# hyye/lio-mapping

Hardware: AMD Instinct MI355X
Metric: sliding-window solves/sec, 64-line 130k-pt scans, window=15 (opt_window=5) (higher is better)
Workload: dtype f64 (solve) / f32 (features); 1 GPU; HDL-64E outdoor_test_config_64, S_outdoor ray-cast scans, window_size=15 opt_window_size=5, one SolveOptimization per step, clouds resident in HBM; n_lidar_residuals=78236, local_map_points=76752, surf_stack_points=19386, parallelism=1 window

## Files before the change

### lio-mapping_amd/csrc/cloud_kernels.h

```cpp
#pragma once
#include <cstdint>

#include "dev.h"

namespace lio {

struct VoxParams {
  float mn[3], mx[3];
  int minb[3], divb[3];
  int overflow;
  int n_valid;
};

struct Affine3f { float m[12]; };

#define LIO_MAX_FRAMES 32

struct ConcatSeg { const float4 *src; int n; int dst_off; int set_intensity; float intensity; Affine3f tf; int identity; };
struct ConcatArgs { ConcatSeg seg[LIO_MAX_FRAMES]; int nseg; int total; };
void launch_transform_concat(const ConcatArgs &a, float4 *dst, hipStream_t s);

void launch_deskew_to_end(float4 *pts, int n, const float q[4], const float p[3], float time_factor, hipStream_t s);

void launch_cloud_bounds(const float4 *pts, int n, DBuf<float> &partial, VoxParams *d_out, hipStream_t s);

class VoxelGridDev {
 public:
  size_t run(const float4 *in, size_t n, float leaf, DBuf<float4> &out, hipStream_t s, VoxParams *host_params = nullptr);
  void launch(const float4 *in, size_t n, float leaf, DBuf<float4> &out, hipStream_t s);
  size_t finish(VoxParams *host_params = nullptr);
  void set_host_signal(bool on) { use_signal_ = on; }
  VoxelGridDev() = default;
  VoxelGridDev(const VoxelGridDev &) = delete;
  VoxelGridDev &operator=(const VoxelGridDev &) = delete;
  ~VoxelGridDev();

 private:
  const float4 *p_in_ = nullptr; size_t p_n_ = 0; DBuf<float4> *p_out_ = nullptr; hipStream_t p_stream_ = nullptr;
  float p_leaf_ = 0.f;
  void enqueue(bool exact);
  int *h_count_ = nullptr;
  VoxParams *h_params_ = nullptr;
  DBuf<float> partial_;
  DBuf<VoxParams> params_;
  DBuf<uint32_t> keys_, keys2_, vals_, vals2_;
  DBuf<int> count_, tile_heads_;
  DBuf<char> tmp_;
  unsigned *h_flag_ = nullptr;
  unsigned seq_ = 0;
  HostSignal sig_{};
  bool use_signal_ = true;
};
bool host_signal_enabled();

struct GridDesc {
  int origin[3];
  int dims[3];
  float inv_cell;
  int n_points;
};

class KnnGrid {
 public:
  void build(const float4 *pts, size_t n, const float mn[3], const float mx[3], float cell, hipStream_t s);
  const float4 *sorted() const { return sorted_.p; }
  const int *cells() const { return cells_.p; }
  const GridDesc &desc() const { return desc_; }

 private:
  GridDesc desc_{};
  DBuf<uint32_t> keys_, keys2_, vals_, vals2_;
  DBuf<float4> sorted_;
  DBuf<int> cells_, cnt_;
  bool cnt_dirty_ = false;
  DBuf<char> tmp_;
};

struct FeatFrame { const float4 *stack; int M; int slot_off; int tf_index; const uint32_t *order = nullptr; };
struct FeatArgs {
  FeatFrame fr[LIO_MAX_FRAMES];
  int nframes;
  int max_M;
  float min_match_sq_dis, min_plane_dis;
  int mapping_mode;
  float fixed_pz[3];
};
void launch_features(const FeatArgs &a, const float *transforms, const float4 *map_sorted, const int *cells, const GridDesc &g,
                     uint8_t *valid, float4 *coef, float *score, const int *skip_flag, hipStream_t s, float4 *abs_coef = nullptr);

void launch_line_features(const float4 *stack, int M, int slot_off, const float *transform, const float fixed_pz[3], float min_match_sq_dis,
                          const float4 *map_sorted, const int *cells, const GridDesc &g, uint8_t *valid, float4 *coef,
                          const int *skip_flag, hipStream_t s);

void launch_knn(const float4 *query, int m, int k, float radius_sq, const float4 *map_sorted, const int *cells, const GridDesc &g,
                int32_t *idx, float *sqd, hipStream_t s);

void launch_map_round(const FeatArgs &surf, const float4 *corner_stack, int Mc, const float *transform, const float4 *corner_map,
                      const int *corner_cells, const GridDesc &corner_grid, const float4 *surf_map, const int *surf_cells,
                      const GridDesc &surf_grid, uint8_t *valid, float4 *coef, float4 *abs_coef, const int *skip_flag, hipStream_t s);

struct SolveSetup {
  float tf[LIO_MAX_FRAMES][8];
  int ntf;
  float odom_T[8];
  int set_odom;
};
struct OdomState;
void launch_solve_setup(const SolveSetup &a, float *d_transforms, OdomState *d_odom, uint8_t *valid, size_t n_valid, hipStream_t s);
// ... 61 lines not shown
```

### lio-mapping_amd/csrc/cloud_kernels.hip

```cpp
#include <cstring>
#include <hip/hip_runtime.h>
#include <rocprim/rocprim.hpp>

#include <cfloat>
#include <climits>

#include "cloud_kernels.h"
#include "cloud_device.h"

namespace lio {

__global__ void k_transform_concat(ConcatArgs a, float4 *__restrict__ dst) {
  int gid = blockIdx.x * blockDim.x + threadIdx.x;
  if (gid >= a.total) return;
  int sidx = 0;
  for (int k = 1; k < a.nseg; ++k)
    if (gid >= a.seg[k].dst_off) sidx = k;
  const ConcatSeg &sg = a.seg[sidx];
  int local = gid - sg.dst_off;
  float4 p = sg.src[local];
  float4 o;
  if (sg.identity) {
    o = p;
  } else {
    const float *m = sg.tf.m;
    o.x = m[0] * p.x + m[1] * p.y + m[2] * p.z + m[3];
    o.y = m[4] * p.x + m[5] * p.y + m[6] * p.z + m[7];
    o.z = m[8] * p.x + m[9] * p.y + m[10] * p.z + m[11];
    o.w = p.w;
  }
  if (sg.set_intensity) o.w = sg.intensity;
  dst[gid] = o;
}

void launch_transform_concat(const ConcatArgs &a, float4 *dst, hipStream_t s) {
  if (a.total <= 0) return;
  hipLaunchKernelGGL(k_transform_concat, dim3(cdiv(a.total, 256)), dim3(256), 0, s, a, dst);
  LIO_HIP(hipGetLastError());
}

__global__ void k_deskew_to_end(float4 *pts, int n, Quat<float> qe, Vec3<float> te, float time_factor) {
// ... 48 lines not shown
  float mn[3] = {FLT_MAX, FLT_MAX, FLT_MAX}, mx[3] = {-FLT_MAX, -FLT_MAX, -FLT_MAX};
  float cnt = 0;
  for (int b = t; b < nb; b += 256) {
    for (int d = 0; d < 3; ++d) { mn[d] = fminf(mn[d], partial[b * 8 + d]); mx[d] = fmaxf(mx[d], partial[b * 8 + 3 + d]); }
    cnt += partial[b * 8 + 6];
  }
  for (int d = 0; d < 3; ++d) { sm[d][t] = mn[d]; sm[3 + d][t] = mx[d]; }
  sm[6][t] = cnt;
  __syncthreads();
  for (int st = 128; st > 0; st >>= 1) {
    if (t < st) {
      for (int d = 0; d < 3; ++d) { sm[d][t] = fminf(sm[d][t], sm[d][t + st]); sm[3 + d][t] = fmaxf(sm[3 + d][t], sm[3 + d][t + st]); }
      sm[6][t] += sm[6][t + st];
    }
    __syncthreads();
  }
  if (t != 0) return;
  for (int d = 0; d < 3; ++d) { mn[d] = sm[d][0]; mx[d] = sm[3 + d][0]; }
  cnt = sm[6][0];
  VoxParams v;
  long long dd[3];
  for (int d = 0; d < 3; ++d) {
    v.mn[d] = mn[d]; v.mx[d] = mx[d];
    dd[d] = (long long)((mx[d] - mn[d]) * inv_leaf) + 1;
    v.minb[d] = int(floorf(mn[d] * inv_leaf));
    int maxb = int(floorf(mx[d] * inv_leaf));
    v.divb[d] = maxb - v.minb[d] + 1;
  }
  v.overflow = (cnt > 0 && dd[0] * dd[1] * dd[2] > (long long)INT_MAX) ? 1 : 0;
  v.n_valid = int(cnt);
  *out = v;
}

__global__ void k_vox_keys(const float4 *__restrict__ pts, int n, float inv_leaf, const VoxParams *__restrict__ vp,
                           uint32_t *__restrict__ keys, uint32_t *__restrict__ vals) {
  int i = blockIdx.x * blockDim.x + threadIdx.x;
  if (i >= n) return;
  float4 p = pts[i];
  uint32_t key = 0xFFFFFFFFu;
  if (finite3(p)) {
    int i0 = int(floorf(p.x * inv_leaf) - float(vp->minb[0]));
    int i1 = int(floorf(p.y * inv_leaf) - float(vp->minb[1]));
    int i2 = int(floorf(p.z * inv_leaf) - float(vp->minb[2]));
    key = uint32_t(i0 + i1 * vp->divb[0] + i2 * vp->divb[0] * vp->divb[1]);
  }
  keys[i] = key;
  vals[i] = uint32_t(i);
}

#define VOX_KEY_THREADS 256
__global__ void __launch_bounds__(VOX_KEY_THREADS) k_vox_keys_abs(const float4 *__restrict__ pts, int n, float inv_leaf, uint32_t *__restrict__ keys,
                                                                 uint32_t *__restrict__ vals, float *__restrict__ partial, int *__restrict__ range_overflow) {
  const int i = blockIdx.x * VOX_KEY_THREADS + threadIdx.x;
  float mn[3] = {FLT_MAX, FLT_MAX, FLT_MAX}, mx[3] = {-FLT_MAX, -FLT_MAX, -FLT_MAX};
  float cnt = 0;
  if (i < n) {
    const float4 p = pts[i];
    uint32_t key = 0xFFFFFFFFu;
    if (finite3(p)) {
      cnt = 1.f;
      mn[0] = mx[0] = p.x; mn[1] = mx[1] = p.y; mn[2] = mx[2] = p.z;
      const float cx = floorf(p.x * inv_leaf), cy = floorf(p.y * inv_leaf), cz = floorf(p.z * inv_leaf);
      if (fabsf(cx) < 1024.f && fabsf(cy) < 1024.f && fabsf(cz) < 511.f) key = (uint32_t(int(cz) + 512) << 22) | (uint32_t(int(cy) + 1024) << 11) | uint32_t(int(cx) + 1024);
      else *range_overflow = 1;
    }
    keys[i] = key;
    vals[i] = uint32_t(i);
  }
  __shared__ float sm[7][VOX_KEY_THREADS / 64];
  const int lane = threadIdx.x & 63, wv = threadIdx.x >> 6;
#pragma unroll
  for (int o = 32; o > 0; o >>= 1) {
    for (int d = 0; d < 3; ++d) { mn[d] = fminf(mn[d], __shfl_xor(mn[d], o, 64)); mx[d] = fmaxf(mx[d], __shfl_xor(mx[d], o, 64)); }
    cnt += __shfl_xor(cnt, o, 64);
  }
  if (lane == 0) { for (int d = 0; d < 3; ++d) { sm[d][wv] = mn[d]; sm[3 + d][wv] = mx[d]; } sm[6][wv] = cnt; }
  __syncthreads();
  if (threadIdx.x < 7) {
    const int t = threadIdx.x;
    float v = sm[t][0];
    for (int w = 1; w < VOX_KEY_THREADS / 64; ++w) v = t < 3 ? fminf(v, sm[t][w]) : (t < 6 ? fmaxf(v, sm[t][w]) : v + sm[t][w]);
    partial[size_t(blockIdx.x) * 8 + t] = v;
  }
}

#define VOX_TILE 256
__device__ __forceinline__ bool vox_is_head(const uint32_t *__restrict__ keys, int i, int n, uint32_t k) {
  return i < n && k != 0xFFFFFFFFu && (i == 0 || keys[i - 1] != k);
}
__global__ void __launch_bounds__(VOX_TILE) k_vox_tile_heads(const uint32_t *__restrict__ keys, int n, int *__restrict__ tile_heads,
                                                             const float *__restrict__ partial, int npartial, float inv_leaf, VoxParams *__restrict__ params) {
  if (blockIdx.x == gridDim.x - 1) {
    if (npartial <= 0) return;
    __shared__ float sm[7][VOX_TILE];
    const int t = threadIdx.x;
    float mn[3] = {FLT_MAX, FLT_MAX, FLT_MAX}, mx[3] = {-FLT_MAX, -FLT_MAX, -FLT_MAX};
    float cnt = 0;
    for (int b = t; b < npartial; b += VOX_TILE) {
      for (int d = 0; d < 3; ++d) { mn[d] = fminf(mn[d], partial[size_t(b) * 8 + d]); mx[d] = fmaxf(mx[d], partial[size_t(b) * 8 + 3 + d]); }
      cnt += partial[size_t(b) * 8 + 6];
    }
    for (int d = 0; d < 3; ++d) { sm[d][t] = mn[d]; sm[3 + d][t] = mx[d]; }
    sm[6][t] = cnt;
    __syncthreads();
    for (int st = VOX_TILE / 2; st > 0; st >>= 1) {
      if (t < st) {
        for (int d = 0; d < 3; ++d) { sm[d][t] = fminf(sm[d][t], sm[d][t + st]); sm[3 + d][t] = fmaxf(sm[3 + d][t], sm[3 + d][t + st]); }
        sm[6][t] += sm[6][t + st];
      }
      __syncthreads();
    }
    if (t != 0) return;
    VoxParams v;
    long long dd[3];
    for (int d = 0; d < 3; ++d) {
      v.mn[d] = sm[d][0]; v.mx[d] = sm[3 + d][0];
// ... 62 lines not shown
    int g = base_i + VOX_TILE;
    while (g < n && keys[g] == k) { const float4 p = pts[vals[g]]; ax += p.x; ay += p.y; az += p.z; ai += p.w; ++g; ++cnt; }
  }
  const float c = float(cnt);
  out[pos] = make_float4(ax / c, ay / c, az / c, ai / c);
}

void launch_cloud_bounds(const float4 *pts, int n, DBuf<float> &partial, VoxParams *d_out, hipStream_t s) {
  const int nb = std::max(1, std::min(cdiv(n, 256), 512));
  partial.reserve(size_t(nb) * 8);
  hipLaunchKernelGGL(k_bounds_partial, dim3(nb), dim3(256), 0, s, pts, n, partial.p);
  hipLaunchKernelGGL(k_bounds_final, dim3(1), dim3(256), 0, s, partial.p, nb, 1.0f, d_out);
  LIO_HIP(hipGetLastError());
}

bool host_signal_enabled() {
  static const bool on = [] { const char *e = std::getenv("LIO_HOST_SIGNAL"); return e ? std::atoi(e) != 0 : true; }();
  return on;
}

void VoxelGridDev::launch(const float4 *in, size_t n, float leaf, DBuf<float4> &out, hipStream_t s) {
  p_in_ = in; p_n_ = n; p_out_ = &out; p_stream_ = s; p_leaf_ = leaf;
  if (n == 0) return;
  enqueue(false);
}

void VoxelGridDev::enqueue(bool exact) {
  const float4 *in = p_in_;
  const size_t n = p_n_;
  DBuf<float4> &out = *p_out_;
  hipStream_t s = p_stream_;
  const int ni = int(n);
  const float inv_leaf = 1.0f / p_leaf_;
  const int nkb = cdiv(ni, VOX_KEY_THREADS);
  partial_.reserve(size_t(std::max(nkb, 512)) * 8);
  params_.reserve(1);
  keys_.reserve(n); keys2_.reserve(n); vals_.reserve(n); vals2_.reserve(n);
  if (count_.cap < 2) { count_.reserve(2); LIO_HIP(hipMemsetAsync(count_.p, 0, count_.cap * sizeof(int), s)); }
  out.reserve(n);
  if (!h_count_) {
    LIO_HIP(hipHostMalloc(reinterpret_cast<void **>(&h_count_), 256, hipHostMallocCoherent));
    static_assert(sizeof(VoxMail) <= 128, "mailbox layout");
    std::memset(h_count_, 0, 256);
    h_params_ = reinterpret_cast<VoxParams *>(h_count_ + 1);
    h_flag_ = reinterpret_cast<unsigned *>(reinterpret_cast<char *>(h_count_) + 128);
  }
  int *d_range = count_.p + 1;
  const bool use_sig = use_signal_ && host_signal_enabled();
  if (!use_sig) LIO_HIP(hipMemsetAsync(d_range, 0, sizeof(int), s));
  int npartial = 0;
  if (exact) {
    const int nb = std::min(cdiv(ni, 256), 512);
    hipLaunchKernelGGL(k_bounds_partial, dim3(nb), dim3(256), 0, s, in, ni, partial_.p);
    hipLaunchKernelGGL(k_bounds_final, dim3(1), dim3(256), 0, s, partial_.p, nb, inv_leaf, params_.p);
    hipLaunchKernelGGL(k_vox_keys, dim3(cdiv(ni, 256)), dim3(256), 0, s, in, ni, inv_leaf, params_.p, keys_.p, vals_.p);
  } else {
    hipLaunchKernelGGL(k_vox_keys_abs, dim3(nkb), dim3(VOX_KEY_THREADS), 0, s, in, ni, inv_leaf, keys_.p, vals_.p, partial_.p, d_range);
    npartial = nkb;
  }
  size_t tmp_bytes = 0;
  LIO_HIP(rocprim::radix_sort_pairs(nullptr, tmp_bytes, keys_.p, keys2_.p, vals_.p, vals2_.p, n, 0, 32, s));
  tmp_.reserve(tmp_bytes + 256);
  LIO_HIP(rocprim::radix_sort_pairs(tmp_.p, tmp_bytes, keys_.p, keys2_.p, vals_.p, vals2_.p, n, 0, 32, s));
  const int ntiles = cdiv(ni, VOX_TILE);
  tile_heads_.reserve(ntiles);
  hipLaunchKernelGGL(k_vox_tile_heads, dim3(ntiles + 1), dim3(VOX_TILE), 0, s, keys2_.p, ni, tile_heads_.p, partial_.p, npartial, inv_leaf, params_.p);
  sig_ = HostSignal();
  if (use_sig) { sig_.flag = h_flag_; sig_.seq = ++seq_; }

  hipLaunchKernelGGL(k_vox_centroids, dim3(ntiles), dim3(VOX_TILE), 0, s, in, keys2_.p, vals2_.p, tile_heads_.p, ni, out.p, count_.p, params_.p, d_range,
                     reinterpret_cast<VoxMail *>(h_count_), sig_);
  LIO_HIP(hipGetLastError());
  if (!sig_.flag) {
    VoxMail *m = reinterpret_cast<VoxMail *>(h_count_);
    LIO_HIP(hipMemcpyAsync(&m->count, count_.p, sizeof(int), hipMemcpyDeviceToHost, s));
    LIO_HIP(hipMemcpyAsync(&m->params, params_.p, sizeof(VoxParams), hipMemcpyDeviceToHost, s));
    LIO_HIP(hipMemcpyAsync(&m->range_overflow, d_range, sizeof(int), hipMemcpyDeviceToHost, s));
  }
}

size_t VoxelGridDev::finish(VoxParams *host_params) {
  if (p_n_ == 0) {
    if (host_params) std::memset(host_params, 0, sizeof(*host_params));
    return 0;
  }
  const VoxMail *m = reinterpret_cast<const VoxMail *>(h_count_);
  bool redone = false;
  for (;;) {
    if (sig_.flag) wait_host_signal(sig_, p_stream_);
    else LIO_HIP(hipStreamSynchronize(p_stream_));
    if (m->range_overflow == 1 && !redone) {
      enqueue(true);
      redone = true;
      continue;
    }
    if (redone) LIO_HIP(hipStreamSynchronize(p_stream_));
    break;
  }
  int count = m->count;
  const VoxParams hp = m->params;
  if (hp.overflow) {
    p_out_->reserve(p_n_);
    LIO_HIP(hipMemcpyAsync(p_out_->p, p_in_, p_n_ * sizeof(float4), hipMemcpyDeviceToDevice, p_stream_));
// ... 29 lines not shown

__global__ void k_cell_place(const float4 *__restrict__ pts, const uint32_t *__restrict__ keys, const uint32_t *__restrict__ slot, int n,
                             const int *__restrict__ starts, float4 *__restrict__ sorted, int *__restrict__ cnt) {
  int i = blockIdx.x * blockDim.x + threadIdx.x;
  if (i >= n) return;
  float4 p = pts[i];
  p.w = __int_as_float(i);
  const uint32_t c = keys[i];
  sorted[starts[c] + int(slot[i])] = p;
  cnt[c] = 0;
}

void KnnGrid::build(const float4 *pts, size_t n, const float mn[3], const float mx[3], float cell, hipStream_t s) {
  desc_.inv_cell = 1.0f / cell;
  desc_.n_points = int(n);
  size_t ncells = 1;
  for (int d = 0; d < 3; ++d) {
    int lo = int(std::floor(mn[d] * desc_.inv_cell)) - 1;
    int hi = int(std::floor(mx[d] * desc_.inv_cell)) + 1;
    desc_.origin[d] = lo;
    desc_.dims[d] = hi - lo + 1;
    ncells *= size_t(desc_.dims[d]);
  }
  if (ncells > (size_t(1) << 30)) throw DeviceError("KnnGrid: cell table too large");
  cells_.reserve(ncells + 1);
  if (cnt_.cap < ncells + 1 || cnt_dirty_) {
    cnt_.reserve(ncells + 1);
    LIO_HIP(hipMemsetAsync(cnt_.p, 0, cnt_.cap * sizeof(int), s));
  }
  cnt_dirty_ = true;
  keys_.reserve(std::max<size_t>(n, 1)); vals_.reserve(std::max<size_t>(n, 1)); sorted_.reserve(std::max<size_t>(n, 1));
  const int ni = int(n);
  if (ni) hipLaunchKernelGGL(k_cell_count, dim3(cdiv(ni, 256)), dim3(256), 0, s, pts, ni, desc_, keys_.p, vals_.p, cnt_.p);
  size_t tmp_bytes = 0;
  LIO_HIP(rocprim::exclusive_scan(nullptr, tmp_bytes, cnt_.p, cells_.p, 0, ncells + 1, rocprim::plus<int>(), s));
  tmp_.reserve(tmp_bytes + 256);
  LIO_HIP(rocprim::exclusive_scan(tmp_.p, tmp_bytes, cnt_.p, cells_.p, 0, ncells + 1, rocprim::plus<int>(), s));
  if (ni) hipLaunchKernelGGL(k_cell_place, dim3(cdiv(ni, 256)), dim3(256), 0, s, pts, keys_.p, vals_.p, ni, cells_.p, sorted_.p, cnt_.p);
  LIO_HIP(hipGetLastError());
  cnt_dirty_ = false;
}

template <int K>
__device__ inline void knn_scan(const Vec3<float> &q, const float4 *__restrict__ map, const int *__restrict__ cells, const GridDesc &g,
                                float (&bd)[K], int (&bi)[K], int (&bj)[K]) {
#pragma unroll
  for (int k = 0; k < K; ++k) { bd[k] = INFINITY; bi[k] = INT_MAX; bj[k] = 0; }
  int cx = cell_coord(q.x, g.inv_cell) - g.origin[0];
  int cy = cell_coord(q.y, g.inv_cell) - g.origin[1];
  int cz = cell_coord(q.z, g.inv_cell) - g.origin[2];
  if (cx < 0 || cy < 0 || cz < 0 || cx >= g.dims[0] || cy >= g.dims[1] || cz >= g.dims[2]) return;
  for (int dz = -1; dz <= 1; ++dz) {
    int z = cz + dz;
    if (z < 0 || z >= g.dims[2]) continue;
    for (int dy = -1; dy <= 1; ++dy) {
      int y = cy + dy;
      if (y < 0 || y >= g.dims[1]) continue;
      int row = g.dims[0] * (y + g.dims[1] * z);
      for (int dx = -1; dx <= 1; ++dx) {
        int x = cx + dx;
        if (x < 0 || x >= g.dims[0]) continue;
        const int c0 = cells[row + x], c1 = cells[row + x + 1];
        for (int j = c0; j < c1; ++j) {
          float4 p = map[j];
          float ddx = p.x - q.x, ddy = p.y - q.y, ddz = p.z - q.z;
          float d = ddx * ddx;
          d += ddy * ddy;
          d += ddz * ddz;
          int idx = __float_as_int(p.w);
          if (d < bd[K - 1] || (d == bd[K - 1] && idx < bi[K - 1])) {
// ... 414 lines not shown
```

### lio-mapping_amd/csrc/seg_sort.hip

```cpp
#include <hip/hip_runtime.h>

#include <algorithm>
#include <cstdlib>
#include <type_traits>
#include <vector>

#include "dev.h"
#include "seg_sort.h"

namespace lio {

#define SS_KEY_NONE_STORED 0x7FFFFFFFu
#define SS_KEY_NONE 0xFFFFFFFFu

__device__ __forceinline__ uint32_t ss_key(uint32_t k, const KeyLayout *__restrict__ L) {
  if (!L) return k;
  if (k == SS_KEY_NONE_STORED) return SS_KEY_NONE;
  const uint32_t x = (k & 2047u) - uint32_t(L->mx), y = ((k >> 11) & 2047u) - uint32_t(L->my), z = (k >> 22) - uint32_t(L->mz);
  return ((z << L->by) | (y << L->bx) | x) & 0x7FFFFFFFu;
}

__device__ __forceinline__ void ss_wave_lds_sync() {
  __builtin_amdgcn_fence(__ATOMIC_RELEASE, "wavefront");
  __builtin_amdgcn_wave_barrier();
  __builtin_amdgcn_fence(__ATOMIC_ACQUIRE, "wavefront");
}

template <int THREADS>
__device__ __forceinline__ int ss_index(int tile, int wave, int round, int lane) { return tile * (THREADS * SS_ITEMS) + wave * (64 * SS_ITEMS) + round * 64 + lane; }

template <int THREADS>
__global__ void __launch_bounds__(THREADS) k_ss_hist(const SegDesc *__restrict__ desc, const uint32_t *__restrict__ keys, uint32_t *__restrict__ hist, int shift, int bits,
                                                     const KeyLayout *__restrict__ layout) {
  const SegDesc sg = desc[blockIdx.y];
  constexpr int TILE = THREADS * SS_ITEMS;
  const int ntiles = (sg.n + TILE - 1) / TILE, tile = blockIdx.x;
  if (tile >= ntiles) return;
  __shared__ uint32_t h[1 << SS_MAX_BITS];
  const int nb = 1 << bits;
  for (int d = threadIdx.x; d < nb; d += THREADS) h[d] = 0;
  __syncthreads();
  const KeyLayout *L = layout ? layout + blockIdx.y : nullptr;
  const int lane = threadIdx.x & 63, wave = threadIdx.x >> 6;
  uint32_t k[SS_ITEMS];
#pragma unroll
  for (int r = 0; r < SS_ITEMS; ++r) {
    const int i = ss_index<THREADS>(tile, wave, r, lane);
    k[r] = i < sg.n ? keys[sg.off + i] : 0u;
  }
#pragma unroll
  for (int r = 0; r < SS_ITEMS; ++r) {
    const int i = ss_index<THREADS>(tile, wave, r, lane);
    if (i < sg.n) atomicAdd(&h[(ss_key(k[r], L) >> shift) & uint32_t(nb - 1)], 1u);
  }
  __syncthreads();
  for (int d = threadIdx.x; d < nb; d += THREADS) hist[size_t(sg.hist_off) + size_t(d) * ntiles + tile] = h[d];
}

// ... 18 lines not shown
  uint32_t base = 0;
  for (int w = 0; w < wave; ++w) base += ws[w];
  uint32_t run = base + incl - sum;
  for (int i = b0; i < b1; ++i) { const uint32_t t = h[i]; h[i] = run; run += t; }
}

template <int THREADS, bool STAGED>
__global__ void __launch_bounds__(THREADS) k_ss_scatter(const SegDesc *__restrict__ desc, const uint32_t *__restrict__ keys_in, const uint32_t *__restrict__ vals_in,
                                                        uint32_t *__restrict__ keys_out, uint32_t *__restrict__ vals_out, const uint32_t *__restrict__ hist, int shift,
                                                        int bits, const KeyLayout *__restrict__ layout) {
  const SegDesc sg = desc[blockIdx.y];
  constexpr int TILE = THREADS * SS_ITEMS, NW = THREADS / 64, NB = 1 << SS_MAX_BITS;
  const int ntiles = (sg.n + TILE - 1) / TILE, tile = blockIdx.x;
  if (tile >= ntiles) return;
  extern __shared__ uint32_t ss_lds[];
  using WH = typename std::conditional<STAGED, uint16_t, uint32_t>::type;
  WH (*wh)[NB] = reinterpret_cast<WH (*)[NB]>(ss_lds);
  uint32_t *delta = ss_lds + NW * NB * sizeof(WH) / 4;
  uint32_t *sk = delta + NB, *sv = sk + TILE;
  const int nb = 1 << bits;
  for (int e = threadIdx.x; e < int(NW * NB * sizeof(WH) / 4); e += THREADS) ss_lds[e] = 0;
  const KeyLayout *L = layout ? layout + blockIdx.y : nullptr;
  const int lane = threadIdx.x & 63, wave = threadIdx.x >> 6;
  uint32_t key[SS_ITEMS], val[SS_ITEMS];
#pragma unroll
  for (int r = 0; r < SS_ITEMS; ++r) {
    const int i = ss_index<THREADS>(tile, wave, r, lane);
    const bool in = i < sg.n;
    key[r] = in ? keys_in[sg.off + i] : 0u;
    val[r] = in ? (vals_in ? vals_in[sg.off + i] : uint32_t(sg.off + i)) : 0u;
  }
  __syncthreads();
  WH *mine = wh[wave];
  const unsigned long long lt = (1ull << lane) - 1ull;
  uint32_t loc[SS_ITEMS];
#pragma unroll
  for (int r = 0; r < SS_ITEMS; ++r) {
    const int i = ss_index<THREADS>(tile, wave, r, lane);
    const bool in = i < sg.n;
    key[r] = ss_key(key[r], L);
    const uint32_t d = (key[r] >> shift) & uint32_t(nb - 1);
    unsigned long long m = __ballot(in);
    for (int b = 0; b < bits; ++b) {
      const bool bit = (d >> b) & 1u;
      const unsigned long long bal = __ballot(bit);
      m &= bit ? bal : ~bal;
    }
    const uint32_t old = in ? mine[d] : 0u;
    ss_wave_lds_sync();
    if (in && (m & lt) == 0ull) mine[d] = WH(old + uint32_t(__popcll(m)));
    ss_wave_lds_sync();
    loc[r] = old + uint32_t(__popcll(m & lt));
  }
  __syncthreads();
  if constexpr (!STAGED) {
    for (int d = threadIdx.x; d < nb; d += THREADS) {
      uint32_t g = hist[size_t(sg.hist_off) + size_t(d) * ntiles + tile];
#pragma unroll
      for (int w = 0; w < NW; ++w) { const uint32_t t = wh[w][d]; wh[w][d] = WH(g); g += t; }
    }
    __syncthreads();
#pragma unroll
    for (int r = 0; r < SS_ITEMS; ++r) {
      const int i = ss_index<THREADS>(tile, wave, r, lane);
      if (i < sg.n) {
        const uint32_t d = (key[r] >> shift) & uint32_t(nb - 1);
        const size_t pos = size_t(sg.off) + mine[d] + loc[r];
        keys_out[pos] = key[r];
        vals_out[pos] = val[r];
      }
    }
  } else {
    constexpr int DPT = (NB + THREADS - 1) / THREADS;
    uint32_t tot[DPT], pre[DPT];
    uint32_t tsum = 0;
#pragma unroll
    for (int q = 0; q < DPT; ++q) {
      const int d = threadIdx.x * DPT + q;
      uint32_t t = 0;
      if (d < nb) for (int w = 0; w < NW; ++w) t += wh[w][d];
      tot[q] = t; pre[q] = tsum; tsum += t;
    }
    uint32_t incl = tsum;
#pragma unroll
    for (int o = 1; o < 64; o <<= 1) { const uint32_t t = __shfl_up(incl, o, 64); if (lane >= o) incl += t; }
// ... 120 lines not shown
```

Measured before the change: 2225 solves/s.

## Replace rocPRIM radix sort and scan with custom onesweep sort and lookback scan

Swaps rocprim::radix_sort_pairs in the voxel grid for a custom 4-pass 8-bit onesweep radix sort with decoupled lookback. The per-digit histograms are computed inside the voxel key kernels, which now loop over several items per thread with a capped grid. The rocprim exclusive scan in the KNN grid build is replaced by a single-pass lookback scan, and the wave-level digit ranking helper is shared with the segmented sort. The goal is to cut launch count, temp-buffer queries and the separate histogram pass, at the cost of spin-wait lookback that relies on forward-progress ticket ordering.

```diff
diff --git a/lio-mapping_amd/csrc/cloud_kernels.h b/lio-mapping_amd/csrc/cloud_kernels.h
--- a/lio-mapping_amd/csrc/cloud_kernels.h
+++ b/lio-mapping_amd/csrc/cloud_kernels.h
@@ -2,6 +2,7 @@
 #include <cstdint>
 
 #include "dev.h"
+#include "radix_sort.h"
 
 namespace lio {
 
@@ -45,7 +46,7 @@
   DBuf<VoxParams> params_;
   DBuf<uint32_t> keys_, keys2_, vals_, vals2_;
   DBuf<int> count_, tile_heads_;
-  DBuf<char> tmp_;
+  RadixSort sort_;
   unsigned *h_flag_ = nullptr;
   unsigned seq_ = 0;
   HostSignal sig_{};
@@ -73,7 +74,7 @@
   DBuf<float4> sorted_;
   DBuf<int> cells_, cnt_;
   bool cnt_dirty_ = false;
-  DBuf<char> tmp_;
+  LookbackScan scan_;
 };
 
 struct FeatFrame { const float4 *stack; int M; int slot_off; int tf_index; const uint32_t *order = nullptr; };
diff --git a/lio-mapping_amd/csrc/cloud_kernels.hip b/lio-mapping_amd/csrc/cloud_kernels.hip
--- a/lio-mapping_amd/csrc/cloud_kernels.hip
+++ b/lio-mapping_amd/csrc/cloud_kernels.hip
@@ -1,12 +1,12 @@
 #include <cstring>
 #include <hip/hip_runtime.h>
-#include <rocprim/rocprim.hpp>
 
 #include <cfloat>
 #include <climits>
 
 #include "cloud_kernels.h"
 #include "cloud_device.h"
+#include "radix_sort.h"
 
 namespace lio {
 
@@ -121,40 +121,68 @@
   *out = v;
 }
 
-__global__ void k_vox_keys(const float4 *__restrict__ pts, int n, float inv_leaf, const VoxParams *__restrict__ vp,
-                           uint32_t *__restrict__ keys, uint32_t *__restrict__ vals) {
-  int i = blockIdx.x * blockDim.x + threadIdx.x;
-  if (i >= n) return;
-  float4 p = pts[i];
-  uint32_t key = 0xFFFFFFFFu;
-  if (finite3(p)) {
-    int i0 = int(floorf(p.x * inv_leaf) - float(vp->minb[0]));
-    int i1 = int(floorf(p.y * inv_leaf) - float(vp->minb[1]));
-    int i2 = int(floorf(p.z * inv_leaf) - float(vp->minb[2]));
-    key = uint32_t(i0 + i1 * vp->divb[0] + i2 * vp->divb[0] * vp->divb[1]);
-  }
-  keys[i] = key;
-  vals[i] = uint32_t(i);
-}
-
 #define VOX_KEY_THREADS 256
+#define VOX_KEY_ITEMS 4
+#define VOX_KEY_MAX_BLOCKS 1024
+static int vox_key_blocks(int n) { return std::max(1, std::min(cdiv(n, VOX_KEY_THREADS * VOX_KEY_ITEMS), VOX_KEY_MAX_BLOCKS)); }
+
+__global__ void __launch_bounds__(VOX_KEY_THREADS) k_vox_keys(const float4 *__restrict__ pts, int n, float inv_leaf, const VoxParams *__restrict__ vp,
+                                                             uint32_t *__restrict__ keys, uint32_t *__restrict__ hist) {
+  __shared__ uint32_t h[RS_PASSES * RS_BINS];
+  for (int e = threadIdx.x; e < RS_PASSES * RS_BINS; e += VOX_KEY_THREADS) h[e] = 0;
+  __syncthreads();
+  for (int b0 = blockIdx.x * (VOX_KEY_THREADS * VOX_KEY_ITEMS); b0 < n; b0 += gridDim.x * (VOX_KEY_THREADS * VOX_KEY_ITEMS)) {
+    float4 p[VOX_KEY_ITEMS];
+#pragma unroll
+    for (int k = 0; k < VOX_KEY_ITEMS; ++k) { const int i = b0 + k * VOX_KEY_THREADS + threadIdx.x; if (i < n) p[k] = pts[i]; }
+#pragma unroll
+    for (int k = 0; k < VOX_KEY_ITEMS; ++k) {
+      const int i = b0 + k * VOX_KEY_THREADS + threadIdx.x;
+      uint32_t key = 0xFFFFFFFFu;
+      if (i < n) {
+        if (finite3(p[k])) {
+          int i0 = int(floorf(p[k].x * inv_leaf) - float(vp->minb[0]));
+          int i1 = int(floorf(p[k].y * inv_leaf) - float(vp->minb[1]));
+          int i2 = int(floorf(p[k].z * inv_leaf) - float(vp->minb[2]));
+          key = uint32_t(i0 + i1 * vp->divb[0] + i2 * vp->divb[0] * vp->divb[1]);
+        }
+        keys[i] = key;
+      }
+      rs_hist_add(h, key, i < n);
+    }
+  }
+  __syncthreads();
+  rs_hist_flush<VOX_KEY_THREADS>(h, hist);
+}
+
 __global__ void __launch_bounds__(VOX_KEY_THREADS) k_vox_keys_abs(const float4 *__restrict__ pts, int n, float inv_leaf, uint32_t *__restrict__ keys,
-                                                                 uint32_t *__restrict__ vals, float *__restrict__ partial, int *__restrict__ range_overflow) {
-  const int i = blockIdx.x * VOX_KEY_THREADS + threadIdx.x;
+                                                                 uint32_t *__restrict__ hist, float *__restrict__ partial, int *__restrict__ range_overflow) {
+  __shared__ uint32_t h[RS_PASSES * RS_BINS];
+  for (int e = threadIdx.x; e < RS_PASSES * RS_BINS; e += VOX_KEY_THREADS) h[e] = 0;
+  __syncthreads();
   float mn[3] = {FLT_MAX, FLT_MAX, FLT_MAX}, mx[3] = {-FLT_MAX, -FLT_MAX, -FLT_MAX};
   float cnt = 0;
-  if (i < n) {
-    const float4 p = pts[i];
-    uint32_t key = 0xFFFFFFFFu;
-    if (finite3(p)) {
-      cnt = 1.f;
-      mn[0] = mx[0] = p.x; mn[1] = mx[1] = p.y; mn[2] = mx[2] = p.z;
-      const float cx = floorf(p.x * inv_leaf), cy = floorf(p.y * inv_leaf), cz = floorf(p.z * inv_leaf);
-      if (fabsf(cx) < 1024.f && fabsf(cy) < 1024.f && fabsf(cz) < 511.f) key = (uint32_t(int(cz) + 512) << 22) | (uint32_t(int(cy) + 1024) << 11) | uint32_t(int(cx) + 1024);
-      else *range_overflow = 1;
-    }
-    keys[i] = key;
-    vals[i] = uint32_t(i);
+  for (int b0 = blockIdx.x * (VOX_KEY_THREADS * VOX_KEY_ITEMS); b0 < n; b0 += gridDim.x * (VOX_KEY_THREADS * VOX_KEY_ITEMS)) {
+    float4 p[VOX_KEY_ITEMS];
+#pragma unroll
+    for (int k = 0; k < VOX_KEY_ITEMS; ++k) { const int i = b0 + k * VOX_KEY_THREADS + threadIdx.x; if (i < n) p[k] = pts[i]; }
+#pragma unroll
+    for (int k = 0; k < VOX_KEY_ITEMS; ++k) {
+      const int i = b0 + k * VOX_KEY_THREADS + threadIdx.x;
+      uint32_t key = 0xFFFFFFFFu;
+      if (i < n) {
+        if (finite3(p[k])) {
+          cnt += 1.f;
+          mn[0] = fminf(mn[0], p[k].x); mn[1] = fminf(mn[1], p[k].y); mn[2] = fminf(mn[2], p[k].z);
+          mx[0] = fmaxf(mx[0], p[k].x); mx[1] = fmaxf(mx[1], p[k].y); mx[2] = fmaxf(mx[2], p[k].z);
+          const float cx = floorf(p[k].x * inv_leaf), cy = floorf(p[k].y * inv_leaf), cz = floorf(p[k].z * inv_leaf);
+          if (fabsf(cx) < 1024.f && fabsf(cy) < 1024.f && fabsf(cz) < 511.f) key = (uint32_t(int(cz) + 512) << 22) | (uint32_t(int(cy) + 1024) << 11) | uint32_t(int(cx) + 1024);
+          else *range_overflow = 1;
+        }
+        keys[i] = key;
+      }
+      rs_hist_add(h, key, i < n);
+    }
   }
   __shared__ float sm[7][VOX_KEY_THREADS / 64];
   const int lane = threadIdx.x & 63, wv = threadIdx.x >> 6;
@@ -171,6 +199,7 @@
     for (int w = 1; w < VOX_KEY_THREADS / 64; ++w) v = t < 3 ? fminf(v, sm[t][w]) : (t < 6 ? fmaxf(v, sm[t][w]) : v + sm[t][w]);
     partial[size_t(blockIdx.x) * 8 + t] = v;
   }
+  rs_hist_flush<VOX_KEY_THREADS>(h, hist);
 }
 
 #define VOX_TILE 256
@@ -299,10 +328,11 @@
   hipStream_t s = p_stream_;
   const int ni = int(n);
   const float inv_leaf = 1.0f / p_leaf_;
-  const int nkb = cdiv(ni, VOX_KEY_THREADS);
+  const int nkb = vox_key_blocks(ni);
   partial_.reserve(size_t(std::max(nkb, 512)) * 8);
   params_.reserve(1);
   keys_.reserve(n); keys2_.reserve(n); vals_.reserve(n); vals2_.reserve(n);
+  uint32_t *hist = sort_.prepare(n, s);
   if (count_.cap < 2) { count_.reserve(2); LIO_HIP(hipMemsetAsync(count_.p, 0, count_.cap * sizeof(int), s)); }
   out.reserve(n);
   if (!h_count_) {
@@ -320,22 +350,19 @@
     const int nb = std::min(cdiv(ni, 256), 512);
     hipLaunchKernelGGL(k_bounds_partial, dim3(nb), dim3(256), 0, s, in, ni, partial_.p);
     hipLaunchKernelGGL(k_bounds_final, dim3(1), dim3(256), 0, s, partial_.p, nb, inv_leaf, params_.p);
-    hipLaunchKernelGGL(k_vox_keys, dim3(cdiv(ni, 256)), dim3(256), 0, s, in, ni, inv_leaf, params_.p, keys_.p, vals_.p);
+    hipLaunchKernelGGL(k_vox_keys, dim3(nkb), dim3(VOX_KEY_THREADS), 0, s, in, ni, inv_leaf, params_.p, keys_.p, hist);
   } else {
-    hipLaunchKernelGGL(k_vox_keys_abs, dim3(nkb), dim3(VOX_KEY_THREADS), 0, s, in, ni, inv_leaf, keys_.p, vals_.p, partial_.p, d_range);
+    hipLaunchKernelGGL(k_vox_keys_abs, dim3(nkb), dim3(VOX_KEY_THREADS), 0, s, in, ni, inv_leaf, keys_.p, hist, partial_.p, d_range);
     npartial = nkb;
   }
-  size_t tmp_bytes = 0;
-  LIO_HIP(rocprim::radix_sort_pairs(nullptr, tmp_bytes, keys_.p, keys2_.p, vals_.p, vals2_.p, n, 0, 32, s));
-  tmp_.reserve(tmp_bytes + 256);
-  LIO_HIP(rocprim::radix_sort_pairs(tmp_.p, tmp_bytes, keys_.p, keys2_.p, vals_.p, vals2_.p, n, 0, 32, s));
+  sort_.sort(keys_.p, vals_.p, keys2_.p, vals2_.p, ni, s);
   const int ntiles = cdiv(ni, VOX_TILE);
   tile_heads_.reserve(ntiles);
-  hipLaunchKernelGGL(k_vox_tile_heads, dim3(ntiles + 1), dim3(VOX_TILE), 0, s, keys2_.p, ni, tile_heads_.p, partial_.p, npartial, inv_leaf, params_.p);
+  hipLaunchKernelGGL(k_vox_tile_heads, dim3(ntiles + 1), dim3(VOX_TILE), 0, s, keys_.p, ni, tile_heads_.p, partial_.p, npartial, inv_leaf, params_.p);
   sig_ = HostSignal();
   if (use_sig) { sig_.flag = h_flag_; sig_.seq = ++seq_; }
 
-  hipLaunchKernelGGL(k_vox_centroids, dim3(ntiles), dim3(VOX_TILE), 0, s, in, keys2_.p, vals2_.p, tile_heads_.p, ni, out.p, count_.p, params_.p, d_range,
+  hipLaunchKernelGGL(k_vox_centroids, dim3(ntiles), dim3(VOX_TILE), 0, s, in, keys_.p, vals_.p, tile_heads_.p, ni, out.p, count_.p, params_.p, d_range,
                      reinterpret_cast<VoxMail *>(h_count_), sig_);
   LIO_HIP(hipGetLastError());
   if (!sig_.flag) {
@@ -431,10 +458,7 @@
   keys_.reserve(std::max<size_t>(n, 1)); vals_.reserve(std::max<size_t>(n, 1)); sorted_.reserve(std::max<size_t>(n, 1));
   const int ni = int(n);
   if (ni) hipLaunchKernelGGL(k_cell_count, dim3(cdiv(ni, 256)), dim3(256), 0, s, pts, ni, desc_, keys_.p, vals_.p, cnt_.p);
-  size_t tmp_bytes = 0;
-  LIO_HIP(rocprim::exclusive_scan(nullptr, tmp_bytes, cnt_.p, cells_.p, 0, ncells + 1, rocprim::plus<int>(), s));
-  tmp_.reserve(tmp_bytes + 256);
-  LIO_HIP(rocprim::exclusive_scan(tmp_.p, tmp_bytes, cnt_.p, cells_.p, 0, ncells + 1, rocprim::plus<int>(), s));
+  scan_.exclusive_scan(cnt_.p, cells_.p, ncells + 1, s);
   if (ni) hipLaunchKernelGGL(k_cell_place, dim3(cdiv(ni, 256)), dim3(256), 0, s, pts, keys_.p, vals_.p, ni, cells_.p, sorted_.p, cnt_.p);
   LIO_HIP(hipGetLastError());
   cnt_dirty_ = false;
diff --git a/lio-mapping_amd/csrc/radix_sort.h b/lio-mapping_amd/csrc/radix_sort.h
--- /dev/null
+++ b/lio-mapping_amd/csrc/radix_sort.h
@@ -0,0 +1,89 @@
+#pragma once
+#include <hip/hip_runtime.h>
+
+#include <cstdint>
+
+#include "dev.h"
+
+namespace lio {
+
+#define RS_BITS 8
+#define RS_BINS (1 << RS_BITS)
+#define RS_PASSES 4
+
+struct RadixSortState {
+  unsigned long long ticket;
+  unsigned done;
+  unsigned pad;
+  uint32_t hist[RS_PASSES][RS_BINS];
+};
+
+class RadixSort {
+ public:
+  uint32_t *prepare(size_t n, hipStream_t s);
+  void sort(uint32_t *keys, uint32_t *vals, uint32_t *keys_tmp, uint32_t *vals_tmp, int n, hipStream_t s);
+
+ private:
+  DBuf<char> state_;
+  RadixSortState *st() const { return reinterpret_cast<RadixSortState *>(state_.p); }
+  DBuf<unsigned long long> status_;
+};
+
+class LookbackScan {
+ public:
+  void exclusive_scan(const int *in, int *out, size_t n, hipStream_t s);
+
+ private:
+  DBuf<unsigned long long> ticket_, status_;
+};
+
+#if defined(__HIPCC__)
+__device__ __forceinline__ void wave_lds_sync() {
+  __builtin_amdgcn_fence(__ATOMIC_RELEASE, "wavefront");
+  __builtin_amdgcn_wave_barrier();
+  __builtin_amdgcn_fence(__ATOMIC_ACQUIRE, "wavefront");
+}
+
+template <typename WH>
+__device__ __forceinline__ uint32_t wave_rank_digit(WH *counts, uint32_t d, int bits, bool in) {
+  const unsigned long long lt = (1ull << (threadIdx.x & 63)) - 1ull;
+  unsigned long long m = __ballot(in);
+  for (int b = 0; b < bits; ++b) {
+    const bool bit = (d >> b) & 1u;
+    const unsigned long long bal = __ballot(bit);
+    m &= bit ? bal : ~bal;
+  }
+  const uint32_t old = in ? uint32_t(counts[d]) : 0u;
+  wave_lds_sync();
+  if (in && (m & lt) == 0ull) counts[d] = WH(old + uint32_t(__popcll(m)));
+  wave_lds_sync();
+  return old + uint32_t(__popcll(m & lt));
+}
+
+__device__ __forceinline__ void rs_hist_add(uint32_t *h, uint32_t key, bool in) {
+  const int lane = threadIdx.x & 63;
+#pragma unroll
+  for (int p = 0; p < RS_PASSES; ++p) {
+    const uint32_t d = (key >> (p * RS_BITS)) & uint32_t(RS_BINS - 1);
+    const unsigned long long act = __ballot(in);
+    bool rest = false;
+    if (act) {
+      const int first = __ffsll((long long)act) - 1;
+      const uint32_t d0 = uint32_t(__builtin_amdgcn_readlane(int(d), first));
+      const unsigned long long m = __ballot(in && d == d0);
+      if (lane == first) atomicAdd(&h[p * RS_BINS + d0], uint32_t(__popcll(m)));
+      rest = in && d != d0;
+    }
+    if (rest) atomicAdd(&h[p * RS_BINS + d], 1u);
+  }
+}
+template <int THREADS>
+__device__ __forceinline__ void rs_hist_flush(const uint32_t *h, uint32_t *ghist) {
+  for (int b = threadIdx.x; b < RS_PASSES * RS_BINS; b += THREADS) {
+    const uint32_t v = h[b];
+    if (v) atomicAdd(&ghist[b], v);
+  }
+}
+#endif
+
+}
diff --git a/lio-mapping_amd/csrc/radix_sort.hip b/lio-mapping_amd/csrc/radix_sort.hip
--- /dev/null
+++ b/lio-mapping_amd/csrc/radix_sort.hip
@@ -0,0 +1,304 @@
+#include <hip/hip_runtime.h>
+
+#include <algorithm>
+
+#include "radix_sort.h"
+
+namespace lio {
+
+#define RS_WINDOW 16
+#define RS_SPIN_LIMIT (1u << 20)
+#define RS_THREADS 1024
+#define RS_ITEMS 4
+#define RS_TILE (RS_THREADS * RS_ITEMS)
+
+__device__ __forceinline__ unsigned long long rs_load(const unsigned long long *p) { return __hip_atomic_load(p, __ATOMIC_RELAXED, __HIP_MEMORY_SCOPE_AGENT); }
+__device__ __forceinline__ void rs_publish(unsigned long long *p, uint32_t tag, uint32_t v) {
+  __hip_atomic_store(p, (static_cast<unsigned long long>(tag) << 32) | v, __ATOMIC_RELAXED, __HIP_MEMORY_SCOPE_AGENT);
+}
+
+__device__ __forceinline__ unsigned long long rs_take_ticket(unsigned long long *ticket, int ntiles) {
+  const unsigned long long t = atomicAdd(ticket, 1ull);
+  if (uint32_t(t) == uint32_t(ntiles - 1)) __hip_atomic_store(ticket, ((t >> 32) + 1ull) << 32, __ATOMIC_RELAXED, __HIP_MEMORY_SCOPE_AGENT);
+  return t;
+}
+
+__device__ uint32_t rs_lookback_lane(const unsigned long long *status, int stride, int tile, uint32_t tag_agg) {
+  const uint32_t tag_inc = tag_agg + 1u;
+  uint32_t sum = 0;
+  int j = tile - 1;
+  unsigned idle = 0;
+  while (j >= 0) {
+    unsigned long long g[RS_WINDOW];
+#pragma unroll
+    for (int k = 0; k < RS_WINDOW; ++k) g[k] = j - k >= 0 ? rs_load(status + size_t(j - k) * stride) : 0ull;
+    int used = 0;
+    bool go = true, fin = false;
+#pragma unroll
+    for (int k = 0; k < RS_WINDOW; ++k) {
+      if (!go) continue;
+      if (j - k < 0) { fin = true; go = false; continue; }
+      const uint32_t tag = uint32_t(g[k] >> 32);
+      if (tag == tag_inc) { sum += uint32_t(g[k]); fin = true; go = false; }
+      else if (tag == tag_agg) { sum += uint32_t(g[k]); ++used; }
+      else go = false;
+    }
+    if (fin) break;
+    j -= used;
+    if (used == 0) {
+      if (++idle > RS_SPIN_LIMIT) break;
+      __builtin_amdgcn_s_sleep(1);
+    }
+  }
+  return sum;
+}
+
+template <int THREADS, int ITEMS>
+__global__ void __launch_bounds__(THREADS) k_rs_pass(const uint32_t *__restrict__ keys_in, const uint32_t *__restrict__ vals_in, uint32_t *__restrict__ keys_out,
+                                                     uint32_t *__restrict__ vals_out, int n, int pass, RadixSortState *st, unsigned long long *status) {
+  constexpr int TILE = THREADS * ITEMS, NW = THREADS / 64;
+  static_assert(THREADS >= RS_BINS && TILE <= 65535, "tile shape");
+  __shared__ uint16_t wh[NW][RS_BINS];
+  __shared__ uint32_t sk[TILE], sv[TILE];
+  __shared__ uint32_t delta[RS_BINS];
+  __shared__ uint32_t wsum[RS_BINS / 64][2];
+  __shared__ unsigned long long s_ticket;
+  __shared__ unsigned s_done;
+  const int tid = threadIdx.x, lane = tid & 63, wave = tid >> 6;
+  const int ntiles = (n + TILE - 1) / TILE;
+  const int shift = pass * RS_BITS;
+  if (tid == 0) s_ticket = rs_take_ticket(&st->ticket, ntiles);
+  for (int e = tid; e < NW * RS_BINS; e += THREADS) (&wh[0][0])[e] = 0;
+  __syncthreads();
+  const int tile = int(uint32_t(s_ticket));
+  if (tile >= ntiles) return;
+  const uint32_t tag_agg = uint32_t(s_ticket >> 32) * 2u + 2u;
+  const int base = tile * TILE + wave * (64 * ITEMS) + lane;
+  const uint32_t gcnt = tid < RS_BINS ? st->hist[pass][tid] : 0u;
+  uint32_t key[ITEMS], val[ITEMS], loc[ITEMS];
+#pragma unroll
+  for (int r = 0; r < ITEMS; ++r) {
+    const int i = base + r * 64;
+    const bool in = i < n;
+    key[r] = in ? keys_in[i] : 0u;
+    val[r] = in ? (vals_in ? vals_in[i] : uint32_t(i)) : 0u;
+  }
+#pragma unroll
+  for (int r = 0; r < ITEMS; ++r) loc[r] = wave_rank_digit(wh[wave], (key[r] >> shift) & uint32_t(RS_BINS - 1), RS_BITS, base + r * 64 < n);
+  __syncthreads();
+  uint32_t tot = 0;
+  if (tid < RS_BINS) {
+#pragma unroll
+    for (int w = 0; w < NW; ++w) tot += wh[w][tid];
+    rs_publish(status + size_t(tile) * RS_BINS + tid, tile == 0 ? tag_agg + 1u : tag_agg, tot);
+  }
+  uint32_t a = tot, b = gcnt;
+#pragma unroll
+  for (int o = 1; o < 64; o <<= 1) {
+    const uint32_t ta = __shfl_up(a, o, 64), tb = __shfl_up(b, o, 64);
+    if (lane >= o) { a += ta; b += tb; }
+  }
+  if (tid < RS_BINS && lane == 63) { wsum[wave][0] = a; wsum[wave][1] = b; }
+  __syncthreads();
+  if (tid < RS_BINS) {
+    uint32_t lstart = a - tot, gstart = b - gcnt;
+    for (int w = 0; w < wave; ++w) { lstart += wsum[w][0]; gstart += wsum[w][1]; }
+    uint32_t l = lstart;
+#pragma unroll
+    for (int w = 0; w < NW; ++w) { const uint32_t t = wh[w][tid]; wh[w][tid] = uint16_t(l); l += t; }
+    uint32_t prefix = 0;
+    if (tile > 0) {
+      prefix = rs_lookback_lane(status + tid, RS_BINS, tile, tag_agg);
+      rs_publish(status + size_t(tile) * RS_BINS + tid, tag_agg + 1u, prefix + tot);
+    }
+    delta[tid] = gstart + prefix - lstart;
+  }
+  __syncthreads();
+#pragma unroll
+  for (int r = 0; r < ITEMS; ++r) {
+    if (base + r * 64 < n) {
+      const uint32_t lp = uint32_t(wh[wave][(key[r] >> shift) & uint32_t(RS_BINS - 1)]) + loc[r];
+      sk[lp] = key[r]; sv[lp] = val[r];
+    }
+  }
+  __syncthreads();
+  const int tile_n = min(TILE, n - tile * TILE);
+  for (int j = tid; j < tile_n; j += THREADS) {
+    const uint32_t k = sk[j];
+    const uint32_t pos = delta[(k >> shift) & uint32_t(RS_BINS - 1)] + uint32_t(j);
+    if (pos < uint32_t(n)) { keys_out[pos] = k; vals_out[pos] = sv[j]; }
+  }
+  if (pass == RS_PASSES - 1) {
+    __syncthreads();
+    if (tid == 0) s_done = atomicAdd(&st->done, 1u);
+    __syncthreads();
+    if (s_done == uint32_t(ntiles - 1)) {
+      for (int e = tid; e < RS_PASSES * RS_BINS; e += THREADS) (&st->hist[0][0])[e] = 0u;
+      if (tid == 0) st->done = 0u;
+    }
+  }
+}
+
+uint32_t *RadixSort::prepare(size_t n, hipStream_t s) {
+  if (n > size_t(INT32_MAX)) throw DeviceError("RadixSort: more than 2^31 - 1 keys");
+  if (!state_.p) {
+    state_.reserve(sizeof(RadixSortState), s);
+    LIO_HIP(hipMemsetAsync(state_.p, 0, sizeof(RadixSortState), s));
+  }
+  const size_t words = std::max<size_t>(cdiv((long long)n, RS_TILE), 1) * RS_BINS;
+  if (status_.cap < words) {
+    status_.reserve(words, s);
+    LIO_HIP(hipMemsetAsync(status_.p, 0, status_.cap * sizeof(unsigned long long), s));
+  }
+  return &st()->hist[0][0];
+}
+
+void RadixSort::sort(uint32_t *keys, uint32_t *vals, uint32_t *keys_tmp, uint32_t *vals_tmp, int n, hipStream_t s) {
+  if (n <= 0) return;
+  uint32_t *ki = keys, *vi = nullptr, *ko = keys_tmp, *vo = vals_tmp;
+  for (int p = 0; p < RS_PASSES; ++p) {
+    hipLaunchKernelGGL((k_rs_pass<RS_THREADS, RS_ITEMS>), dim3(cdiv(n, RS_TILE)), dim3(RS_THREADS), 0, s, ki, vi, ko, vo, n, p, st(), status_.p);
+    std::swap(ki, ko);
+    vi = vo;
+    vo = (vo == vals_tmp) ? vals : vals_tmp;
+  }
+  LIO_HIP(hipGetLastError());
+}
+
+#define SC_THREADS 512
+#define SC_VEC 4
+#define SC_TILE (SC_THREADS * SC_VEC * 4)
+#define SC_LOOK 4
+
+__device__ uint32_t sc_lookback_wave(const unsigned long long *status, int tile, uint32_t tag_agg) {
+  const uint32_t tag_inc = tag_agg + 1u;
+  const int lane = threadIdx.x & 63;
+  constexpr int SPAN = SC_LOOK * 64;
+  uint32_t sum = 0;
+  int j = tile - 1;
+  unsigned idle = 0;
+  while (j >= 0) {
+    unsigned long long g[SC_LOOK];
+#pragma unroll
+    for (int k = 0; k < SC_LOOK; ++k) { const int jj = j - (k * 64 + lane); g[k] = jj >= 0 ? rs_load(status + jj) : 0ull; }
+    int first_inc = SPAN, first_nr = SPAN;
+#pragma unroll
+    for (int k = 0; k < SC_LOOK; ++k) {
+      const int dist = k * 64 + lane;
+      const uint32_t tag = uint32_t(g[k] >> 32);
+      if (j - dist < 0 || tag == tag_inc) first_inc = min(first_inc, dist);
+      else if (tag != tag_agg) first_nr = min(first_nr, dist);
+    }
+#pragma unroll
+    for (int o = 32; o > 0; o >>= 1) { first_inc = min(first_inc, __shfl_xor(first_inc, o, 64)); first_nr = min(first_nr, __shfl_xor(first_nr, o, 64)); }
+    const bool fin = first_inc < first_nr;
+    const int upto = fin ? first_inc + 1 : first_nr;
+    uint32_t part = 0;
+#pragma unroll
+    for (int k = 0; k < SC_LOOK; ++k) {
+      const int dist = k * 64 + lane;
+      if (dist < upto && j - dist >= 0) part += uint32_t(g[k]);
+    }
+#pragma unroll
+    for (int o = 32; o > 0; o >>= 1) part += __shfl_xor(part, o, 64);
+    sum += part;
+    if (fin) break;
+    j -= first_nr;
+    if (first_nr == 0) {
+      if (++idle > RS_SPIN_LIMIT) break;
+      __builtin_amdgcn_s_sleep(1);
+    }
+  }
+  return sum;
+}
+
+__global__ void __launch_bounds__(SC_THREADS) k_lookback_scan(const int *__restrict__ in, int *__restrict__ out, long long n, unsigned long long *ticket,
+                                                              unsigned long long *status) {
+  constexpr int NW = SC_THREADS / 64;
+  __shared__ unsigned long long s_ticket;
+  __shared__ uint32_t wsum[SC_VEC][NW];
+  __shared__ uint32_t s_prefix;
+  const int tid = threadIdx.x, lane = tid & 63, wave = tid >> 6;
+  const int ntiles = int((n + SC_TILE - 1) / SC_TILE);
+  if (tid == 0) s_ticket = rs_take_ticket(ticket, ntiles);
+  __syncthreads();
+  const int tile = int(uint32_t(s_ticket));
+  if (tile >= ntiles) return;
+  const uint32_t tag_agg = uint32_t(s_ticket >> 32) * 2u + 2u;
+  const long long base = (long long)tile * SC_TILE;
+  int4 v[SC_VEC];
+  uint32_t incl[SC_VEC], own[SC_VEC];
+#pragma unroll
+  for (int c = 0; c < SC_VEC; ++c) {
+    const long long i = base + 4ll * (c * SC_THREADS + tid);
+    if (i + 3 < n) v[c] = *reinterpret_cast<const int4 *>(in + i);
+    else {
+      v[c].x = i < n ? in[i] : 0; v[c].y = i + 1 < n ? in[i + 1] : 0; v[c].z = i + 2 < n ? in[i + 2] : 0; v[c].w = 0;
+    }
+    own[c] = uint32_t(v[c].x) + uint32_t(v[c].y) + uint32_t(v[c].z) + uint32_t(v[c].w);
+    incl[c] = own[c];
+  }
+#pragma unroll
+  for (int o = 1; o < 64; o <<= 1) {
+#pragma unroll
+    for (int c = 0; c < SC_VEC; ++c) { const uint32_t t = __shfl_up(incl[c], o, 64); if (lane >= o) incl[c] += t; }
+  }
+  if (lane == 63) {
+#pragma unroll
+    for (int c = 0; c < SC_VEC; ++c) wsum[c][wave] = incl[c];
+  }
+  __syncthreads();
+  uint32_t start[SC_VEC], total = 0;
+#pragma unroll
+  for (int c = 0; c < SC_VEC; ++c) {
+    uint32_t before = 0, col = 0;
+#pragma unroll
+    for (int w = 0; w < NW; ++w) { const uint32_t t = wsum[c][w]; col += t; if (w < wave) before += t; }
+    start[c] = total + before + incl[c] - own[c];
+    total += col;
+  }
+  if (wave == 0) {
+    if (lane == 0) rs_publish(status + tile, tile == 0 ? tag_agg + 1u : tag_agg, total);
+    uint32_t prefix = 0;
+    if (tile > 0) {
+      prefix = sc_lookback_wave(status, tile, tag_agg);
+      if (lane == 0) rs_publish(status + tile, tag_agg + 1u, prefix + total);
+    }
+    if (lane == 0) s_prefix = prefix;
+  }
+  __syncthreads();
+  const uint32_t prefix = s_prefix;
+#pragma unroll
+  for (int c = 0; c < SC_VEC; ++c) {
+    const long long i = base + 4ll * (c * SC_THREADS + tid);
+    int4 o;
+    o.x = int(prefix + start[c]);
+    o.y = o.x + v[c].x;
+    o.z = o.y + v[c].y;
+    o.w = o.z + v[c].z;
+    if (i + 3 < n) *reinterpret_cast<int4 *>(out + i) = o;
+    else {
+      if (i < n) out[i] = o.x;
+      if (i + 1 < n) out[i + 1] = o.y;
+      if (i + 2 < n) out[i + 2] = o.z;
+    }
+  }
+}
+
+void LookbackScan::exclusive_scan(const int *in, int *out, size_t n, hipStream_t s) {
+  if (n == 0) return;
+  if (n > size_t(INT32_MAX)) throw DeviceError("LookbackScan: more than 2^31 - 1 elements");
+  const size_t ntiles = (n + SC_TILE - 1) / SC_TILE;
+  if (!ticket_.p) {
+    ticket_.reserve(1, s);
+    LIO_HIP(hipMemsetAsync(ticket_.p, 0, sizeof(unsigned long long), s));
+  }
+  if (status_.cap < ntiles) {
+    status_.reserve(ntiles, s);
+    LIO_HIP(hipMemsetAsync(status_.p, 0, status_.cap * sizeof(unsigned long long), s));
+  }
+  hipLaunchKernelGGL(k_lookback_scan, dim3(unsigned(ntiles)), dim3(SC_THREADS), 0, s, in, out, (long long)n, ticket_.p, status_.p);
+  LIO_HIP(hipGetLastError());
+}
+
+}
diff --git a/lio-mapping_amd/csrc/seg_sort.hip b/lio-mapping_amd/csrc/seg_sort.hip
--- a/lio-mapping_amd/csrc/seg_sort.hip
+++ b/lio-mapping_amd/csrc/seg_sort.hip
@@ -6,6 +6,7 @@
 #include <vector>
 
 #include "dev.h"
+#include "radix_sort.h"
 #include "seg_sort.h"
 
 namespace lio {
@@ -18,12 +19,6 @@
   if (k == SS_KEY_NONE_STORED) return SS_KEY_NONE;
   const uint32_t x = (k & 2047u) - uint32_t(L->mx), y = ((k >> 11) & 2047u) - uint32_t(L->my), z = (k >> 22) - uint32_t(L->mz);
   return ((z << L->by) | (y << L->bx) | x) & 0x7FFFFFFFu;
-}
-
-__device__ __forceinline__ void ss_wave_lds_sync() {
-  __builtin_amdgcn_fence(__ATOMIC_RELEASE, "wavefront");
-  __builtin_amdgcn_wave_barrier();
-  __builtin_amdgcn_fence(__ATOMIC_ACQUIRE, "wavefront");
 }
 
 template <int THREADS>
@@ -108,25 +103,13 @@
   }
   __syncthreads();
   WH *mine = wh[wave];
-  const unsigned long long lt = (1ull << lane) - 1ull;
   uint32_t loc[SS_ITEMS];
 #pragma unroll
   for (int r = 0; r < SS_ITEMS; ++r) {
     const int i = ss_index<THREADS>(tile, wave, r, lane);
     const bool in = i < sg.n;
     key[r] = ss_key(key[r], L);
-    const uint32_t d = (key[r] >> shift) & uint32_t(nb - 1);
-    unsigned long long m = __ballot(in);
-    for (int b = 0; b < bits; ++b) {
-      const bool bit = (d >> b) & 1u;
-      const unsigned long long bal = __ballot(bit);
-      m &= bit ? bal : ~bal;
-    }
-    const uint32_t old = in ? mine[d] : 0u;
-    ss_wave_lds_sync();
-    if (in && (m & lt) == 0ull) mine[d] = WH(old + uint32_t(__popcll(m)));
-    ss_wave_lds_sync();
-    loc[r] = old + uint32_t(__popcll(m & lt));
+    loc[r] = wave_rank_digit(mine, (key[r] >> shift) & uint32_t(nb - 1), bits, in);
   }
   __syncthreads();
   if constexpr (!STAGED) {
```

Measured after the change: 2286 solves/s (median of 6 runs). 1.03x the previous value.
